# uricchio/2DSFS-scan

Measured on NVIDIA B200. Metric: SNPs/sec, 2D-SFS + T2D/T1D 20 kb window scan, higher is better.
Workload: dtype u32 popcount/histograms + f64 likelihoods

## Files before the change

2dsfs-scan_b200/csrc/tdsfs.cu:

```cuda
#include <algorithm>
#include <cmath>
#include <cstdarg>
#include <cstdio>
#include <cstdlib>
#include <cstring>
#include <string>
#include <vector>

#include <nvtx3/nvToolsExt.h>

#include "tdsfs_kernels.cuh"
#include "tdsfs_fused.cuh"

using namespace tdsfs;

#define TDSFS_VERSION 200

static thread_local std::string g_err;

struct NvtxRange {
  explicit NvtxRange(const char* name) { nvtxRangePushA(name); }
  ~NvtxRange() { nvtxRangePop(); }
};

// ... 70 lines not shown
  double* d_ws = nullptr;
  long long ws_cap = 0;
  long long fused_W = -1;
  int fused_snp = -1;
  bool ws_ready = false;
  bool last_fused = false;
  double* d_dxI = nullptr;
  int bg_mode = -1, NG = 0;
  long long gstride = 0;
  uint32_t* d_hist = nullptr;
  long long hist_words = 0;
  int32_t* d_bg_group = nullptr;
  int32_t* d_score_group = nullptr;
  bool per_chrom_scoring = false;
  double *d_lb2 = nullptr, *d_lb1a = nullptr, *d_lb1b = nullptr, *d_B = nullptr, *d_lnI = nullptr;
  unsigned long long* d_Bsum = nullptr;
  int table_groups = 0;
  bool float_bg = false, tables_ready = false, fin_timed = false;
  bool poisson_bg = false;
  double pq_n = 0, pq_sum = 0, pq_lnsum = 0;
  bool tables_from_exchange = false;
  unsigned int* d_gridbar = nullptr;
  unsigned long long* d_stamps = nullptr;
  bool want_tail_exchange = false;
  bool x_timed = false;
  int score_group_warps = 1;
  int* d_err = nullptr;
  int peer_rank = -1, peer_world = 0;
  uint32_t* peer_hist[PEER_MAX] = {};
  unsigned long long* peer_flags[PEER_MAX] = {};
  unsigned long long* d_peer_flags = nullptr;
  uint32_t* peer_exported_hist = nullptr;
  long long peer_words = 0;
  unsigned long long peer_epoch = 0;
  bool peer_ready = false;
  unsigned long long peer_pending = 0;
  long long ncand = 0, cand_cap = 0;
  std::vector<long long> cand_off_host;
  long long cand_W = -1;
  int cand_snp = -1;
  int groups_mode = -1, groups_chrom = -1;
  cudaStream_t plan_stream = nullptr;
  cudaEvent_t ev_fork = nullptr, ev_plan = nullptr, ev_plan0 = nullptr;
  long long plan_W = -1;
  int plan_snp = -1;
  bool planned_last = false;
// ... 78 lines not shown
  c->device = device;
  c->sm_count = prop.multiProcessorCount;
  CK(cudaStreamCreateWithFlags(&c->own_stream, cudaStreamNonBlocking));
  CK(cudaStreamCreateWithFlags(&c->copy_stream, cudaStreamNonBlocking));
  CK(cudaStreamCreateWithFlags(&c->plan_stream, cudaStreamNonBlocking));
  CK(cudaEventCreateWithFlags(&c->ev_fork, cudaEventDisableTiming));
  CK(cudaEventCreate(&c->ev_plan));
  CK(cudaEventCreate(&c->ev_plan0));
  c->stream = c->own_stream;
  for (int i = 0; i < NEV; ++i) CK(cudaEventCreate(&c->ev[i]));
  CKR(dev_alloc(&c->d_err, 1));
  CKR(dev_alloc(&c->d_nlarge, 1));
  CKR(dev_alloc(&c->d_lnI, LN_TABLE));
  CK(cudaMemsetAsync(c->d_err, 0, sizeof(int), c->stream));
  k_ln_int_table<<<(LN_TABLE + 255) / 256, 256, 0, c->stream>>>(c->d_lnI, LN_TABLE);
  c->launches++;
  CK(cudaGetLastError());
  CKR(dev_alloc(&c->d_gridbar, 2));
  CK(cudaMemsetAsync(c->d_gridbar, 0, 2 * sizeof(unsigned int), c->stream));
  if (getenv("TDSFS_TAIL_STAMPS")) {
    CKR(dev_alloc(&c->d_stamps, 8));
    CK(cudaMemsetAsync(c->d_stamps, 0, 8 * sizeof(unsigned long long), c->stream));
  }
  CKR(dev_alloc(&c->d_dxI, LN_TABLE));
  k_dx_table<<<(LN_TABLE + 255) / 256, 256, 0, c->stream>>>(c->d_dxI, LN_TABLE);
  c->launches++;
  CK(cudaGetLastError());
  CK(cudaStreamSynchronize(c->stream));
  *out = c;
  return 0;
}

static int pool_get(void** pool, size_t* cap, size_t bytes, void** out) {
  if (bytes > *cap) {
    if (*pool) cudaFree(*pool);
    *pool = nullptr;
    *cap = 0;
    CK(cudaMalloc(pool, std::max<size_t>(bytes, 256)));
    *cap = std::max<size_t>(bytes, 256);
  }
  *out = *pool;
  return 0;
}

static void drop_step_graph(tdsfs_ctx* c) {
  if (c->step_exec) cudaGraphExecDestroy(c->step_exec);
// ... 24 lines not shown
  if (!c) return;
  cudaSetDevice(c->device);
  cudaStreamSynchronize(c->stream);
  drop_step_graph(c);
  free_data(c);
  if (c->pool_G) cudaFree(c->pool_G);
  if (c->pool_cnt) cudaFree(c->pool_cnt);
  if (c->pool_pos) cudaFree(c->pool_pos);
  if (c->pool_flags) cudaFree(c->pool_flags);
  if (c->pool_off) cudaFree(c->pool_off);
  if (c->pool_tmp) cudaFree(c->pool_tmp);
  peer_unmap(c);
  dev_free(c->d_peer_flags);
  dev_free(c->d_work);
  if (c->d_rec) cudaFree(c->d_rec);
  dev_free(c->d_hist); dev_free(c->d_bg_group); dev_free(c->d_score_group);
  dev_free(c->d_lb2); dev_free(c->d_lb1a); dev_free(c->d_lb1b); dev_free(c->d_B); dev_free(c->d_Bsum); dev_free(c->d_lnI);
  dev_free(c->d_err); dev_free(c->d_cand_off); dev_free(c->d_wlo); dev_free(c->d_whi); dev_free(c->d_wchrom);
  dev_free(c->d_large); dev_free(c->d_wstart); dev_free(c->d_wend); dev_free(c->d_nlarge);
  dev_free(c->r_count); dev_free(c->r_n2); dev_free(c->r_n1a); dev_free(c->r_n1b); dev_free(c->r_T2); dev_free(c->r_T1a);
  dev_free(c->r_T1b); dev_free(c->r_flags); dev_free(c->d_scratch);
  for (int i = 0; i < NEV; ++i) if (c->ev[i]) cudaEventDestroy(c->ev[i]);
  dev_free(c->d_dxI); dev_free(c->d_ws); dev_free(c->d_gridbar); dev_free(c->d_stamps);
  cudaStreamDestroy(c->own_stream);
  cudaStreamDestroy(c->copy_stream);
  cudaStreamDestroy(c->plan_stream);
  cudaEventDestroy(c->ev_fork); cudaEventDestroy(c->ev_plan); cudaEventDestroy(c->ev_plan0);
  delete c;
}

extern "C" int tdsfs_set_stream(tdsfs_t* c, void* s) {
  if (!c) return fail(TDSFS_ERR_ARG, "ctx is NULL");
  c->stream = s ? (cudaStream_t)s : c->own_stream;
  drop_step_graph(c);
  return 0;
}

extern "C" int tdsfs_set_sync(tdsfs_t* c, int sync) {
  if (!c) return fail(TDSFS_ERR_ARG, "ctx is NULL");
  c->sync = sync != 0;
  return 0;
}

extern "C" int tdsfs_set_panel(tdsfs_t* c, int32_t n1, int32_t n2, int32_t fold) {
  if (!c) return fail(TDSFS_ERR_ARG, "ctx is NULL");
  if (n1 < 1 || n2 < 1 || n1 > 32767 || n2 > 32767) return fail(TDSFS_ERR_ARG, "panel sizes must be in [1, 32767] (got %d, %d)", n1, n2);
// ... 356 lines not shown
            dev_free(c->d_ws);
            CKR(dev_alloc(&c->d_ws, ncand * 4));
            c->ws_cap = ncand;
          }
          q.W = (uint32_t)c->plan_W;
          q.Wmagic = (uint32_t)std::min<unsigned long long>(0xFFFFFFFFull, (1ull << 32) / (unsigned long long)c->plan_W);
          q.cand_off = c->d_cand_off;
          q.ncand = ncand;
          q.ws = c->d_ws;
          q.dxI = c->d_dxI;
          q.lnI = c->d_lnI;
        } else {
          q.nw1 = q.nw2 = 0;
        }
        q.pos_tma = (((uintptr_t)c->dPos) & 15) == 0 && !getenv("TDSFS_NO_POS_TMA");
        q.snap_nearest = getenv("TDSFS_SNAP_BACK") ? 0 : 1;
        const int per_warp_fixed = q.tab_words * 4;
        while (depth > 1 && p.cwarps * (depth * (stage_stride + 8) + per_warp_fixed) + hist_words * 4 + 16 > smem_max) --depth;
        p.nstage = p.cwarps * depth;
        const int smem = p.nstage * stage_stride + p.cwarps * q.tab_words * 4 + ((p.nstage + 1) & ~1) * 8 + hist_words * 4;
        if (smem > smem_max) return fail(TDSFS_ERR_ARG, "count kernel geometry needs %d bytes of shared memory (warps %d, depth %d)", smem, p.cwarps, depth);
        const bool plain = !c->dFlags && c->nfix == 0 && p.bg_group == nullptr && p.bg_lo < 0 && c->fold && c->fmt.narrow &&
                           c->n1 >= 32 && c->n2 >= 32 && c->n1 <= 1023 && c->n2 <= 1023 && !getenv("TDSFS_NO_PLAIN");
        void (*kern)(FusedParams) = plain ? k1_fused<0, 0, true> : k1_fused<0, 0, false>;
        if (plain && c->W1 == 32 && c->W2 == 32) kern = k1_fused<32, 32, true>;
        else if (plain && c->W1 == 14 && c->W2 == 14) kern = k1_fused<14, 14, true>;
        CK(cudaFuncSetAttribute(kern, cudaFuncAttributeMaxDynamicSharedMemorySize, smem));
        const bool one_launch = c->chunks.size() == 1 && !c->chunks[0].ev && c->chunks[0].r1 > c->chunks[0].r0;
        const bool tail_x = c->want_tail_exchange && one_launch && mode != TDSFS_BG_NONE && NG == 1 && c->peer_ready &&
                            c->d_hist == c->peer_exported_hist && c->gstride == c->peer_words;
        const bool tail_fin = one_launch && mode != TDSFS_BG_NONE && !getenv("TDSFS_NO_TAIL") &&
                              (tail_x || (!c->want_tail_exchange && getenv("TDSFS_TAIL") != nullptr));
        if (tail_fin) {
          CKR(ensure_tables(c, NG));
          q.tail = tail_x ? 2 : 1;
          q.gridbar = c->d_gridbar;
          q.tail_timeout = PEER_TIMEOUT_CYCLES;
          q.stamps = c->d_stamps;
          FinParams& f = q.fin;
          f.hist = c->d_hist; f.gstride = c->gstride; f.NG = NG; f.bins2d = c->bins2d; f.R1 = c->R1; f.R2 = c->R2;
          f.n1 = c->n1; f.n2 = c->n2; f.lb2 = c->d_lb2; f.lb1a = c->d_lb1a; f.lb1b = c->d_lb1b; f.Bsum = c->d_Bsum; f.B = c->d_B;
          if (tail_x) {
            for (int r = 0; r < PEER_MAX; ++r) { q.peer.hist[r] = c->peer_hist[r]; q.peer.flags[r] = c->peer_flags[r]; }
            q.peer.rank = c->peer_rank; q.peer.world = c->peer_world; q.peer.words = c->peer_words; q.peer.err = c->d_err;
            q.peer.timeout_cycles = PEER_TIMEOUT_CYCLES;
            q.peer.ticket = reinterpret_cast<unsigned int*>(c->d_peer_flags + PEER_MAX);
            q.epoch_mem = c->d_peer_flags + PEER_MAX + 1;
            c->peer_epoch += 2;
          }
        }
        const long long tile_rows = (long long)p.tile_blocks * BLK;
        for (auto& ch : c->chunks) {
          if (ch.r1 <= ch.r0) continue;
          if (ch.ev) CK(cudaStreamWaitEvent(st, ch.ev, 0));
          p.r0 = ch.r0; p.r1 = ch.r1;
          const long long ntiles = (ch.r1 - ch.r0 + tile_rows - 1) / tile_rows;
          const int grid = (int)std::max<long long>(1, std::min<long long>((ntiles + p.cwarps - 1) / p.cwarps, (long long)c->sm_count));
          q.k = p;
          kern<<<grid, p.cwarps * 32, smem, st>>>(q);
          c->launches++;
        }
        if (fuse) {
          c->fused_W = c->plan_W;
          c->fused_snp = c->plan_snp;
          c->ws_ready = true;
        }
        if (tail_fin) {
          c->tables_ready = true;
          c->tables_from_exchange = true;
          c->fin_timed = false;
        }
      }
    }
  } else {
    p.r0 = 0; p.r1 = c->S;
    const long long ntiles = (c->S + K1C_THREADS - 1) / K1C_THREADS;
    if (ntiles > 0) {
      CK(cudaFuncSetAttribute(k1_counts, cudaFuncAttributeMaxDynamicSharedMemorySize, hist_bytes));
      const int grid = (int)std::min<long long>(ntiles, (long long)c->sm_count * 4);
      k1_counts<<<grid, K1C_THREADS, hist_bytes, st>>>(p);
      c->launches++;
    }
  }
// ... 730 lines not shown
    cudaEventElapsedTime(&c->ms[3], c->ev[EV_K2], c->ev[EV_K3S]);
    cudaEventElapsedTime(&c->ms[4], c->ev[EV_K3S], c->ev[EV_K3L]);
    cudaEventElapsedTime(&c->ms[6], c->ev[EV_SC0], c->ev[EV_K3L]);
    if (c->keys_ready) cudaEventElapsedTime(&c->ms[7], c->ev[EV_BG0], c->ev[EV_K3L]);
  }
  c->ms[5] = c->ms[0];
  if (c->x_timed) cudaEventElapsedTime(&c->ms[8], c->ev[EV_X0], c->ev[EV_X1]);
  cudaGetLastError();
  for (int i = 0; i < n && i < 10; ++i) ms[i] = c->ms[i];
  return 0;
}

extern "C" int64_t tdsfs_launch_count(tdsfs_t* c) { return c ? c->launches : 0; }

extern "C" int tdsfs_tail_stamps(tdsfs_t* c, uint64_t* out8) {
  if (!c || !out8) return fail(TDSFS_ERR_ARG, "ctx or out is NULL");
  if (!c->d_stamps) return fail(TDSFS_ERR_STATE, "tail stamps are off (create the handle with TDSFS_TAIL_STAMPS=1 set)");
  CK(cudaSetDevice(c->device));
  CK(cudaStreamSynchronize(c->stream));
  CK(cudaMemcpy(out8, c->d_stamps, 8 * sizeof(uint64_t), cudaMemcpyDeviceToHost));
  return 0;
}

extern "C" int tdsfs_scan_info(tdsfs_t* c, int32_t* fused, int32_t* record_bytes) {
  if (!c) return fail(TDSFS_ERR_ARG, "ctx is NULL");
  if (fused) *fused = c->last_fused ? 1 : 0;
  if (record_bytes) *record_bytes = c->fmt.narrow ? 4 : 8;
  return 0;
}
```

2dsfs-scan_b200/csrc/tdsfs_fused.cuh:

```cuda
#pragma once
#include <type_traits>

#include "tdsfs_kernels.cuh"

namespace tdsfs {

constexpr uint32_t WS_ONE_2D = 1u << 10, WS_ONE_1A = 1u << 11, WS_ONE_1B = 1u << 12, WS_NALL = 1u << 13;

struct FusedParams {
  KeyParams k;
  int wmode;
  uint32_t W, Wmagic;
  const long long* cand_off;
  long long ncand;
  double* ws;
  const double* dxI;
  const double* lnI;
  int pos_tma;
  int tab_words;
  int nw1, nw2;
  int snap_nearest;
  int tail;
  unsigned int* gridbar;
  long long tail_timeout;
  FinParams fin;
  PeerParams peer;
  unsigned long long* epoch_mem;
  unsigned long long* stamps;
};

__global__ void k_dx_table(double* t, int n) {
  int i = blockIdx.x * blockDim.x + threadIdx.x;
  if (i < n) t[i] = i ? log((double)i + 1.0) + (double)i * log1p(1.0 / (double)i) : 0.0;
}

__device__ __forceinline__ uint32_t udiv_magic(uint32_t x, uint32_t W, uint32_t M) {
  uint32_t qd = __umulhi(x, M);
  if (x - qd * W >= W) ++qd;
  return qd;
}

struct ChromWin {
  int c = -1, lo = 0, hi = -1;
  int cbase = 0;
  int nfull = 0;
};

__device__ __forceinline__ void chrom_win(const FusedParams& q, int s, ChromWin& cw) {
  if (s >= cw.lo && s < cw.hi) return;
  const KeyParams& p = q.k;
  int lo = 0, hi = p.C;
  while (hi - lo > 1) {
// ... 113 lines not shown
    hi[i] = blk[(2 * i + 1) * BLK];
    both[i] = lo[i] & hi[i];
  }
  const uint32_t c = popc_sum<P>(both);
  alt = popc_sum<P>(lo) + c;
  miss = popc_sum<P>(hi) - c;
}

__device__ __forceinline__ uint32_t fold_fast(int a, int n) {
  const uint32_t f = (uint32_t)min(a, 2 * n - a);
  return (f - 1u) < (uint32_t)(n - 1) ? f : 0u;
}

__device__ __forceinline__ void red_shared_inc_if(bool pr, const uint32_t* base, uint32_t idx) {
  asm volatile("{\n\t.reg .pred p;\n\tsetp.ne.u32 p, %0, 0;\n\t@p red.shared.add.u32 [%1], 1;\n\t}" ::"r"((uint32_t)pr), "r"(smem_u32(base) + idx * 4u) : "memory");
}
__device__ __forceinline__ void red_global_inc_if(bool pr, uint32_t* addr) {
  asm volatile("{\n\t.reg .pred p;\n\tsetp.ne.u32 p, %0, 0;\n\t@p red.global.add.u32 [%1], 1;\n\t}" ::"r"((uint32_t)pr), "l"(addr) : "memory");
}

template <int TW1, int TW2>
constexpr int k1f_max_warps() { return (TW1 + TW2) >= 48 ? 16 : K1_CWARPS; }

template <int TW1, int TW2, bool PLAIN>
__global__ void __launch_bounds__(k1f_max_warps<TW1, TW2>() * 32, 1) k1_fused(const __grid_constant__ FusedParams q) {
  const KeyParams& p = q.k;
  extern __shared__ __align__(128) uint8_t smem[];
  const int tid = threadIdx.x, lane = tid & 31;
  const int warp = __shfl_sync(0xffffffffu, tid >> 5, 0);
  const int W1 = TW1 > 0 ? TW1 : p.W1, W2 = TW2 > 0 ? TW2 : p.W2;
  const int RW = W1 + W2;
  const int tile_rows = p.tile_blocks * BLK;
  const int stage_stride = p.stage_bytes + tile_rows * 4;
  const int depth = p.nstage / p.cwarps;
  uint64_t* full = reinterpret_cast<uint64_t*>(smem + (size_t)p.nstage * stage_stride);
  SinkSmem sm;
  sm.corner = reinterpret_cast<uint32_t*>(full + ((p.nstage + 1) & ~1));
  sm.h1a = sm.corner + p.cr * p.cc;
  sm.h1b = sm.h1a + p.h1a;
  const int nhist = p.cr * p.cc + p.h1a + p.h1b;
  uint32_t* tab = sm.corner + ((nhist + 3) & ~3) + (size_t)warp * q.tab_words;
  uint32_t* w1a = tab + HASH_SLOTS;
  uint32_t* w1b = w1a + q.nw1;

  if (tid == 0) {
    for (int i = 0; i < p.nstage; ++i) mbar_init(full + i, 1);
    fence_barrier_init();
    if (q.stamps && blockIdx.x == 0) q.stamps[0] = (unsigned long long)clock64();
  }
  for (int i = tid; i < nhist; i += blockDim.x) sm.corner[i] = 0;
  if (q.wmode && warp < p.cwarps) {
    for (int i = lane; i < HASH_SLOTS; i += 32) tab[i] = EMPTY_KEY;
    for (int i = lane; i < q.nw1 + q.nw2; i += 32) w1a[i] = 0;
  }
  __syncthreads();

  const int r0 = (int)p.r0, r1 = (int)p.r1, S = (int)p.S;
  const int nparts = gridDim.x * p.cwarps;
  auto target = [&](int jj) -> int {
    if (jj <= 0) return r0;
    if (jj >= nparts) return r1;
    const long long t = r0 + (long long)(r1 - r0) * jj / nparts;
    return max(r0, (int)(t / tile_rows * tile_rows));
  };
  ChromCache cc;
  const int cta_group = PLAIN ? p.uniform_group : tile_group(p, target(blockIdx.x * p.cwarps), cc);

  if (warp < p.cwarps) {
    const int j = blockIdx.x * p.cwarps + warp;
    bool st0 = true, st1 = true, stl = true, sth = true;
    const int lo_clamp = r0 > 0 ? snap_row(q, r0, stl, lane, false) : 0;
    const int hi_clamp = r1 < S ? snap_row(q, r1, sth, lane, false) : S;
    int slo = lo_clamp, shi = hi_clamp;
    if (j > 0) {
      slo = snap_row(q, target(j), st0, lane, q.snap_nearest != 0);
      if (slo <= lo_clamp) { slo = lo_clamp; st0 = stl; }
      if (slo >= hi_clamp) { slo = hi_clamp; st0 = sth; }
    } else {
      st0 = stl;
    }
    if (j + 1 < nparts) {
      shi = snap_row(q, target(j + 1), st1, lane, q.snap_nearest != 0);
      if (shi <= lo_clamp) shi = lo_clamp;
      if (shi >= hi_clamp) shi = hi_clamp;
    }
    slo = __shfl_sync(0xffffffffu, slo, 0);
    shi = __shfl_sync(0xffffffffu, shi, 0);
    st0 = __shfl_sync(0xffffffffu, (int)st0, 0) != 0;
    if (slo < shi) {
      uint8_t* stages = smem + (size_t)warp * depth * stage_stride;
      uint64_t* bars = full + warp * depth;
      const long long block_words = (long long)RW * BLK;
      const int b_end = (r1 + BLK - 1) / BLK;
      const int S4 = S & ~3;
      const int t_begin = slo / tile_rows, t_end = (shi - 1) / tile_rows + 1;
      const int t_whole = min(b_end, S4 / BLK) / p.tile_blocks;
      const uint32_t gbytes_whole = (uint32_t)(p.tile_blocks * block_words * 4);
      const uint32_t pbytes_whole = q.pos_tma ? (uint32_t)tile_rows * 4u : 0u;
      auto issue = [&](int t, int slot) {
        const int blk0 = t * p.tile_blocks;
        uint32_t gbytes = gbytes_whole, pbytes = pbytes_whole;
        if (t >= t_whole) {
          const int nb = min(p.tile_blocks, b_end - blk0);
          gbytes = (uint32_t)(nb * block_words * 4);
          pbytes = q.pos_tma ? (uint32_t)max(0, min(nb * BLK, S4 - blk0 * BLK)) * 4u : 0u;
        }
        uint8_t* stage = stages + (size_t)slot * stage_stride;
        mbar_arrive_expect_tx(bars + slot, gbytes + pbytes);
        bulk_g2s_stream(stage, p.G + (long long)blk0 * block_words, gbytes, bars + slot);
        if (pbytes) bulk_g2s(stage + p.stage_bytes, p.pos + (long long)blk0 * BLK, pbytes, bars + slot);
      };
      if (lane == 0)
        for (int d = 0; d < depth; ++d)
          if (t_begin + d < t_end) issue(t_begin + d, d);
      int slot = 0;
      uint32_t ph = 0;

      int cur_id = -2;
      bool overflow = false;
      bool pending_skip = !st0;
      int wcount = 0;
      int win_end_pos = 0, win_end_row = 0;
      double w2 = 0.0;
      uint32_t nn = 0;
      uint32_t aux = 0;
      ChromWin cw;
      const uint32_t last = (uint32_t)p.bins2d - 1;
      constexpr uint32_t F10 = (1u << KEY_SHIFT) - 1;

      auto close_window = [&]() {
        __syncwarp();
        if (cur_id >= 0) {
          if (!overflow) {
            double a1 = 0.0, b1 = 0.0;
            uint32_t dd = 0;
            for (int i = lane; i < q.nw1; i += 32) {
              const uint32_t v = w1a[i];
// ... 76 lines not shown
          int pv = 0;
          if (live) {
            const uint32_t* rowp = tile + (size_t)b * block_words + lane;
            if constexpr (TW1 > 0 && TW2 > 0) {
              count_pop_planes<TW1>(rowp, T1, M1);
              count_pop_planes<TW2>(rowp + TW1 * BLK, T2, M2);
              T1 += M1;
              T2 += M2;
            } else {
              count_block_b32<TW1>(rowp, W1, T1, M1);
              count_block_b32<TW2>(rowp + W1 * BLK, W2, T2, M2);
            }
            if (q.wmode == 1 && q.pos_tma) {
              if (INTERIOR || s < S4) pv = spos[b * BLK + lane];
              else if (s < S) pv = __ldg(p.pos + s);
            }
          }
          if (q.wmode == 1 && !q.pos_tma) {
            pv = pv_next;
            pv_next = s + BLK < S ? __ldg(p.pos + s + BLK) : 0;
          }
          if (b == nb - 1) {
            __syncwarp();
            if (lane == 0 && t + depth < t_end) {
              fence_proxy_async();
              issue(t + depth, slot);
            }
          }
          if (!live) return;
          const bool whole = INTERIOR || (sb >= slo && sb + BLK <= shi);
          const bool act = whole || (s >= slo && s < shi);
          uint32_t key = 0, fa = 0, fb = 0, cf = 1;
          if (act) {
            const int alt1 = (int)(T1 - M1), alt2 = (int)(T2 - M2);
            const int ref1 = 2 * (p.ns1 - (int)M1) - alt1, ref2 = 2 * (p.ns2 - (int)M2) - alt2;
            if (PLAIN) {
              const bool swapped = alt1 + alt2 > p.n1 + p.n2;
              const int k1 = swapped ? ref1 : alt1, k2 = swapped ? ref2 : alt2;
              int d1 = swapped ? (p.n1 - p.ns1) + (int)M1 : 0, d2 = swapped ? (p.n2 - p.ns2) + (int)M2 : 0;
              if ((d1 | d2) >> p.fmt.md) {
                atomicOr(p.err, 8);
                d1 = d2 = 0;
              }
              key = (uint32_t)(k1 * p.C2 + k2);
              __stcs(reinterpret_cast<uint32_t*>(p.rec) + s,
                     (uint32_t)k1 | ((uint32_t)k2 << p.fmt.b1) | ((uint32_t)d1 << (p.fmt.b1 + p.fmt.b2)) |
                         ((uint32_t)d2 << (p.fmt.b1 + p.fmt.b2 + p.fmt.md)));
              fa = fold_fast(alt1, p.n1);
              fb = fold_fast(alt2, p.n2);
// ... 41 lines not shown
              if (wcount > WCAP) overflow = true;
              else if (mine) insert(key, fa, fb, cf);
            }
          }
          {
            const uint32_t am = __ballot_sync(0xffffffffu, act);
            const int src = 31 - __clz((int)am);
            const int c_lo = __shfl_sync(0xffffffffu, cw.lo, src), c_hi = __shfl_sync(0xffffffffu, cw.hi, src);
            const int c_base = __shfl_sync(0xffffffffu, cw.cbase, src);
            if (cur_id < 0) {
              win_end_pos = 0;
              win_end_row = 0;
            } else if (q.wmode == 1) {
              const long long e = 1 + (long long)(cur_id - c_base + 1) * (long long)q.W;
              win_end_pos = e > 0x7FFFFFFFLL ? 0x7FFFFFFF : (int)e;
              win_end_row = c_hi;
            } else {
              win_end_pos = 0x7FFFFFFF;
              win_end_row = c_lo + (cur_id - c_base + 1) * (int)q.W;
            }
          }
      };

      for (int t = t_begin; t < t_end; ++t) {
        const int blk0 = t * p.tile_blocks;
        const int nb = min(p.tile_blocks, b_end - blk0);
        mbar_wait(bars + slot, ph);
        const uint8_t* stage = stages + (size_t)slot * stage_stride;
        const uint32_t* tile = reinterpret_cast<const uint32_t*>(stage);
        const int* spos = reinterpret_cast<const int*>(stage + p.stage_bytes);
        if (blk0 * BLK >= slo && (blk0 + nb) * BLK <= shi) {
          for (int b = 0; b < nb; ++b) do_block(std::true_type{}, t, blk0, nb, b, tile, spos);
        } else {
          for (int b = 0; b < nb; ++b) do_block(std::false_type{}, t, blk0, nb, b, tile, spos);
        }
        if (++slot == depth) { slot = 0; ph ^= 1; }
      }
      if (q.wmode) close_window();
    }
  }
  __syncthreads();
  sink_flush(p, sm, cta_group, tid, blockDim.x);
  if (q.tail) {
    auto stamp = [&](int i) { if (q.stamps && blockIdx.x == 0 && tid == 0) q.stamps[i] = (unsigned long long)clock64(); };
    stamp(1);
    grid_barrier(q.gridbar, p.err, q.tail_timeout);
    stamp(2);
    if (q.tail == 2) peer_exchange(q.peer, q.epoch_mem, q.stamps);
    for (int g = 0; g < q.fin.NG; ++g) finalize_tables(q.fin, g, blockIdx.x, gridDim.x);
    stamp(6);
    finalize_totals(q.fin, gridDim.x);
    stamp(7);
  }
}

struct FinishParams {
  ScoreParams s;
  const double* ws;
  int use_smem;
  int large_ctas;
};

__device__ __forceinline__ uint32_t bin_of(const uint2 r, int which, uint32_t last) {
  if (which == 0) return (r.x != 0 && r.x != last) ? r.x : 0u;
// ... 89 lines not shown
    auto lookup1 = [&](uint32_t rr, double& la, double& lb) {
      const uint32_t k1 = rr & m1, k2 = (rr >> sh2) & m2;
      la = s_a[k1 + 2u * ((rr >> shd1) & md)];
      lb = s_b[k2 + 2u * (rr >> shd2)];
    };
    {
      constexpr int Q = 8;
      auto bounds = [&](long long w, int& lo, int& cnt) {
        lo = 0; cnt = 0;
        if (w < p.ncand) {
          lo = __ldg(p.wlo + w);
          const int c = __ldg(p.whi + w) - lo;
          cnt = c <= WCAP ? c : 0;
        }
      };
      auto load_batch = [&](uint32_t (&r)[Q], int lo, int cnt, int base) {
#pragma unroll
        for (int j = 0; j < Q; ++j) {
          const int i = base + j * 32 + lane;
          r[j] = i < cnt ? __ldcs(rec + lo + i) : 0u;
        }
      };
      double g2 = 0.0, g1a = 0.0, g1b = 0.0;
      auto consume = [&](const uint32_t (&r)[Q]) {
#pragma unroll
        for (int h4 = 0; h4 < Q; h4 += 4) {
          double l2[4], la[4], lb[4];
#pragma unroll
          for (int j = 0; j < 4; ++j) {
            l2[j] = lookup2(r[h4 + j]);
            lookup1(r[h4 + j], la[j], lb[j]);
          }
#pragma unroll
          for (int j = 0; j < 4; ++j) { g2 += l2[j]; g1a += la[j]; g1b += lb[j]; }
        }
      };
      long long id = wid, nid = wid + nwarp;
      int lo, cnt, nlo, ncnt;
      bounds(id, lo, cnt);
      bounds(nid, nlo, ncnt);
      uint32_t rn[Q];
      load_batch(rn, lo, cnt, 0);
      while (id < p.ncand) {
        uint32_t r[Q], r2[Q];
#pragma unroll
        for (int j = 0; j < Q; ++j) r[j] = rn[j];
        if (cnt > Q * 32) load_batch(r2, lo, cnt, Q * 32);
        const long long nnid = nid + nwarp;
        int nnlo, nncnt;
        bounds(nnid, nnlo, nncnt);
        load_batch(rn, nlo, ncnt, 0);
        if (cnt > 0) {
          const double wsv = __ldg(q.ws + id * 4 + (lane & 3));
          g2 = g1a = g1b = 0.0;
          consume(r);
          if (cnt > Q * 32) consume(r2);
          if (cnt > 2 * Q * 32) {
            load_batch(r2, lo, cnt, 2 * Q * 32);
            consume(r2);
          }
          g2 = warp_sum(g2); g1a = warp_sum(g1a); g1b = warp_sum(g1b);
          finish_window(p, id, lo, cnt, g2, g1a, g1b, wsv, p.lb2, p.lb1a, p.lb1b, p.B, lane);
        }
        id = nid; lo = nlo; cnt = ncnt;
        nid = nnid; nlo = nnlo; ncnt = nncnt;
      }
    }
  } else {
    for (long long id = wid; id < p.ncand; id += nwarp) {
      const int lo = __ldg(p.wlo + id), hi = __ldg(p.whi + id);
      const int cnt = hi - lo;
      if (cnt == 0 || cnt > WCAP) continue;
      const int g = p.score_group ? __ldg(p.score_group + __ldg(p.wchrom + id)) : 0;
      const double* lb2 = p.lb2 + (long long)g * p.bins2d;
      const double* lb1a = p.lb1a + (long long)g * (p.n1 + 1);
      const double* lb1b = p.lb1b + (long long)g * (p.n2 + 1);
      double g2 = 0.0, g1a = 0.0, g1b = 0.0;
      constexpr int Q = 4;
      for (int base = 0; base < cnt; base += Q * 32) {
        uint2 r[Q];
        double l2[Q], la[Q], lb[Q];
#pragma unroll
// ... 24 lines not shown
```

2dsfs-scan_b200/tdsfs_capi.py:

```python
from __future__ import annotations

import ctypes as C
import os

import numpy as np

HERE = os.path.dirname(os.path.abspath(__file__))
LIB_PATH = os.path.join(HERE, "lib", "libtdsfs.so")

BG_NONE, BG_PER_CHROM, BG_GENOME, BG_CHROM = 0, 1, 2, 3
F_T2D_NONE, F_T1D_P1_NONE, F_T1D_P2_NONE, F_EMPTY, F_SKIPPED = 1, 2, 4, 8, 16
ERR_ARG, ERR_CUDA, ERR_STATE, ERR_RANGE, ERR_RETRY = 1, 2, 3, 4, 5

EXPORTS = [
    "tdsfs_create", "tdsfs_destroy", "tdsfs_last_error", "tdsfs_set_stream", "tdsfs_set_sync", "tdsfs_set_panel",
    "tdsfs_load_counts", "tdsfs_load_genotypes", "tdsfs_background", "tdsfs_background_device", "tdsfs_get_background",
    "tdsfs_set_background", "tdsfs_finalize_background", "tdsfs_plan_bp", "tdsfs_plan_snp", "tdsfs_candidates_bp", "tdsfs_candidates_snp", "tdsfs_scan_bp",
    "tdsfs_scan_snp", "tdsfs_set_poisson_background", "tdsfs_scan_poisson_bp", "tdsfs_fetch_results", "tdsfs_check", "tdsfs_run_bp", "tdsfs_step_bp", "tdsfs_window_spectra", "tdsfs_likelihood",
    "tdsfs_poisson_score", "tdsfs_peer_export", "tdsfs_peer_import", "tdsfs_peer_allreduce_background", "tdsfs_peer_reduce_finalize", "tdsfs_peer_close",
    "tdsfs_synth_genotypes", "tdsfs_timings", "tdsfs_launch_count", "tdsfs_scan_info", "tdsfs_tail_stamps", "tdsfs_version",
]


PEER_BLOB_BYTES = 192


class TdsfsError(RuntimeError):
    def __init__(self, code, msg):
        super().__init__(f"libtdsfs error {code}: {msg}")
        self.code = code


class Fixup(C.Structure):
    _fields_ = [("snp", C.c_int64), ("pop", C.c_int32), ("dref", C.c_int32), ("dalt", C.c_int32)]


FIXUP_DTYPE = np.dtype([("snp", "<i8"), ("pop", "<i4"), ("dref", "<i4"), ("dalt", "<i4")], align=True)


class Result(C.Structure):
    _fields_ = [("chrom", C.c_void_p), ("start", C.c_void_p), ("end", C.c_void_p), ("snp_count", C.c_void_p),
                ("n2d", C.c_void_p), ("n1d_p1", C.c_void_p), ("n1d_p2", C.c_void_p), ("T2D", C.c_void_p),
                ("T1D_p1", C.c_void_p), ("T1D_p2", C.c_void_p), ("flags", C.c_void_p)]
# ... 228 lines not shown
        self._check(self._L.tdsfs_synth_genotypes(self._h, C.c_void_p(G_dev_ptr), C.c_int64(S), C.c_int64(snp0), C.c_int32(words1),
                                                  C.c_int32(words2), C.c_int32(ns1), C.c_int32(ns2), C.c_uint64(seed),
                                                  C.c_double(missing_rate), C.c_double(fst)))

    def timings(self):
        ms = (C.c_float * 10)()
        self._check(self._L.tdsfs_timings(self._h, ms, C.c_int32(10)))
        names = ["k1_count", "finalize", "k2_bounds", "k3_small", "k3_large", "background_call", "scan_call", "pass_total", "exchange"]
        return dict(zip(names, list(ms)))

    def launch_count(self):
        return int(self._L.tdsfs_launch_count(self._h))

    def scan_info(self):
        f, b = C.c_int32(), C.c_int32()
        self._check(self._L.tdsfs_scan_info(self._h, C.byref(f), C.byref(b)))
        return bool(f.value), int(b.value)

    def tail_stamps(self):
        out = (C.c_uint64 * 8)()
        self._check(self._L.tdsfs_tail_stamps(self._h, out))
        return [int(x) for x in out]

    def check(self):
        self._check(self._L.tdsfs_check(self._h))
```

include/tdsfs.h:

```cpp
#ifndef TDSFS_H
#define TDSFS_H

#include <stdint.h>

#ifdef __cplusplus
extern "C" {
#endif

typedef struct tdsfs_ctx tdsfs_t;

enum {
  TDSFS_OK = 0,
  TDSFS_ERR_ARG = 1,
  TDSFS_ERR_CUDA = 2,
  TDSFS_ERR_STATE = 3,
  TDSFS_ERR_RANGE = 4,
  TDSFS_ERR_RETRY = 5
};

enum {
  TDSFS_F_T2D_NONE = 1,
  TDSFS_F_T1D_P1_NONE = 2,
  TDSFS_F_T1D_P2_NONE = 4,
  TDSFS_F_EMPTY = 8,
// ... 71 lines not shown
int tdsfs_fetch_results(tdsfs_t* ctx, tdsfs_result_t* out, int64_t cap, int64_t* n_windows);

int tdsfs_check(tdsfs_t* ctx);

int tdsfs_run_bp(tdsfs_t* ctx, int32_t bg_mode, int64_t W, tdsfs_result_t* out, int64_t cap, int64_t* n_windows);

int tdsfs_set_poisson_background(tdsfs_t* ctx, const double* q2d);
int tdsfs_scan_poisson_bp(tdsfs_t* ctx, int64_t W, tdsfs_result_t* out, int64_t cap, int64_t* n_windows);

int tdsfs_step_bp(tdsfs_t* ctx, int32_t bg_mode, int64_t W);

int tdsfs_window_spectra(tdsfs_t* ctx, int64_t window, uint64_t* sfs2d, uint64_t* sfs1d_p1, uint64_t* sfs1d_p2);

int tdsfs_likelihood(tdsfs_t* ctx, const int64_t* x, const double* b, int64_t n, double B, double* T, int32_t* flag);

int tdsfs_poisson_score(tdsfs_t* ctx, const int64_t* x, const double* mu, int64_t n, double* score);

int tdsfs_synth_genotypes(tdsfs_t* ctx, void* G_dev, int64_t S, int64_t snp0, int32_t words1, int32_t words2,
                          int32_t ns1, int32_t ns2, uint64_t seed, double missing_rate, double fst);
int tdsfs_timings(tdsfs_t* ctx, float* ms, int32_t n);
int64_t tdsfs_launch_count(tdsfs_t* ctx);
int tdsfs_scan_info(tdsfs_t* ctx, int32_t* fused, int32_t* record_bytes);
int tdsfs_tail_stamps(tdsfs_t* ctx, uint64_t* out8);
int tdsfs_version(void);

#ifdef __cplusplus
}
#endif
#endif
```

Baseline: 22.42 billion.

## Add dynamic tail work-stealing to fused count kernel via atomic chunk pool

The fused count kernel now splits its row range into a static part (about 85% by default) that is divided evenly across warps, plus a pool of shrinking chunks that warps claim through a global atomic counter once their static range is done. Chunk bounds are snapped to window boundaries and cached in a tagged global array, and the next chunk's first tile is prefetched at the end of the current one. A per-launch epoch counter resets the pool. The aim is to cut load imbalance at the tail of the scan, at the cost of extra atomics, window-state resets and a second kernel instantiation. The likelihood consume loop also skips unused batch groups, and optional per-CTA timing stamps are added for profiling.

```diff
diff --git a/2dsfs-scan_b200/csrc/tdsfs.cu b/2dsfs-scan_b200/csrc/tdsfs.cu
--- a/2dsfs-scan_b200/csrc/tdsfs.cu
+++ b/2dsfs-scan_b200/csrc/tdsfs.cu
@@ -116,6 +116,11 @@
   bool tables_from_exchange = false;
   unsigned int* d_gridbar = nullptr;
   unsigned long long* d_stamps = nullptr;
+  unsigned int* d_k1dyn = nullptr;
+  unsigned long long* d_k1bnd = nullptr;
+  long long k1bnd_cap = 0;
+  unsigned long long* d_cta_stamps = nullptr;
+  int cta_stamps_n = 0;
   bool want_tail_exchange = false;
   bool x_timed = false;
   int score_group_warps = 1;
@@ -240,6 +245,12 @@
     CKR(dev_alloc(&c->d_stamps, 8));
     CK(cudaMemsetAsync(c->d_stamps, 0, 8 * sizeof(unsigned long long), c->stream));
   }
+  CKR(dev_alloc(&c->d_k1dyn, 4));
+  CK(cudaMemsetAsync(c->d_k1dyn, 0, 4 * sizeof(unsigned int), c->stream));
+  if (getenv("TDSFS_K1_STAMPS")) {
+    CKR(dev_alloc(&c->d_cta_stamps, 2 * (long long)c->sm_count));
+    CK(cudaMemsetAsync(c->d_cta_stamps, 0, 2 * (size_t)c->sm_count * sizeof(unsigned long long), c->stream));
+  }
   CKR(dev_alloc(&c->d_dxI, LN_TABLE));
   k_dx_table<<<(LN_TABLE + 255) / 256, 256, 0, c->stream>>>(c->d_dxI, LN_TABLE);
   c->launches++;
@@ -310,6 +321,7 @@
   dev_free(c->r_T1b); dev_free(c->r_flags); dev_free(c->d_scratch);
   for (int i = 0; i < NEV; ++i) if (c->ev[i]) cudaEventDestroy(c->ev[i]);
   dev_free(c->d_dxI); dev_free(c->d_ws); dev_free(c->d_gridbar); dev_free(c->d_stamps);
+  dev_free(c->d_k1dyn); dev_free(c->d_k1bnd); dev_free(c->d_cta_stamps);
   cudaStreamDestroy(c->own_stream);
   cudaStreamDestroy(c->copy_stream);
   cudaStreamDestroy(c->plan_stream);
@@ -712,10 +724,16 @@
         if (smem > smem_max) return fail(TDSFS_ERR_ARG, "count kernel geometry needs %d bytes of shared memory (warps %d, depth %d)", smem, p.cwarps, depth);
         const bool plain = !c->dFlags && c->nfix == 0 && p.bg_group == nullptr && p.bg_lo < 0 && c->fold && c->fmt.narrow &&
                            c->n1 >= 32 && c->n2 >= 32 && c->n1 <= 1023 && c->n2 <= 1023 && !getenv("TDSFS_NO_PLAIN");
-        void (*kern)(FusedParams) = plain ? k1_fused<0, 0, true> : k1_fused<0, 0, false>;
-        if (plain && c->W1 == 32 && c->W2 == 32) kern = k1_fused<32, 32, true>;
-        else if (plain && c->W1 == 14 && c->W2 == 14) kern = k1_fused<14, 14, true>;
-        CK(cudaFuncSetAttribute(kern, cudaFuncAttributeMaxDynamicSharedMemorySize, smem));
+        void (*kerns[2])(FusedParams) = {plain ? k1_fused<0, 0, true, false> : k1_fused<0, 0, false, false>,
+                                         plain ? k1_fused<0, 0, true, true> : k1_fused<0, 0, false, true>};
+        if (plain && c->W1 == 32 && c->W2 == 32) {
+          kerns[0] = k1_fused<32, 32, true, false>;
+          kerns[1] = k1_fused<32, 32, true, true>;
+        } else if (plain && c->W1 == 14 && c->W2 == 14) {
+          kerns[0] = k1_fused<14, 14, true, false>;
+          kerns[1] = k1_fused<14, 14, true, true>;
+        }
+        for (auto kn : kerns) CK(cudaFuncSetAttribute(kn, cudaFuncAttributeMaxDynamicSharedMemorySize, smem));
         const bool one_launch = c->chunks.size() == 1 && !c->chunks[0].ev && c->chunks[0].r1 > c->chunks[0].r0;
         const bool tail_x = c->want_tail_exchange && one_launch && mode != TDSFS_BG_NONE && NG == 1 && c->peer_ready &&
                             c->d_hist == c->peer_exported_hist && c->gstride == c->peer_words;
@@ -740,15 +758,50 @@
           }
         }
         const long long tile_rows = (long long)p.tile_blocks * BLK;
+        constexpr double K1_DYN_MIN_WINDOWS = 16.0;
+        const char* e_static = getenv("TDSFS_K1_STATIC");
+        const int k1_mode = depth != 1 ? 1 : (e_static ? (atoi(e_static) != 0 ? 1 : 0) : -1);
+        const long long ncand_all = q.wmode ? c->cand_off_host[c->C] : 0;
+        double static_frac = 0.85;
+        if (const char* e = getenv("TDSFS_K1_STATIC_FRAC")) static_frac = std::max(0.0, std::min(1.0, atof(e)));
+        int chunk_tiles = 0;
+        if (const char* e = getenv("TDSFS_K1_CHUNK")) chunk_tiles = std::max(0, atoi(e));
+        q.cta_stamps = c->d_cta_stamps;
         for (auto& ch : c->chunks) {
           if (ch.r1 <= ch.r0) continue;
           if (ch.ev) CK(cudaStreamWaitEvent(st, ch.ev, 0));
           p.r0 = ch.r0; p.r1 = ch.r1;
           const long long ntiles = (ch.r1 - ch.r0 + tile_rows - 1) / tile_rows;
           const int grid = (int)std::max<long long>(1, std::min<long long>((ntiles + p.cwarps - 1) / p.cwarps, (long long)c->sm_count));
+          q.pool_lo = (int)ch.r1;
+          q.nchunk = 0;
+          q.chunk_tiles = chunk_tiles;
+          const double rows_per_win = ncand_all > 0 ? (double)c->S / (double)ncand_all : 0.0;
+          const double win_per_warp = rows_per_win > 0.0 ? (double)(ch.r1 - ch.r0) / rows_per_win / ((double)grid * p.cwarps) : 0.0;
+          if (k1_mode == 0 || (k1_mode < 0 && win_per_warp >= K1_DYN_MIN_WINDOWS)) {
+            const long long pool_lo = std::max<long long>(ch.r0, (ch.r0 + (long long)(static_frac * (double)(ch.r1 - ch.r0))) / tile_rows * tile_rows);
+            const long long pool_tiles = (ch.r1 - pool_lo + tile_rows - 1) / tile_rows;
+            long long m = std::min<long long>(pool_tiles, 2LL * grid * p.cwarps);
+            if (rows_per_win > 0.0) m = std::min<long long>(m, std::max<long long>(1, (long long)((double)(ch.r1 - pool_lo) / (4.0 * rows_per_win))));
+            if (chunk_tiles > 0) m = (pool_tiles + chunk_tiles - 1) / chunk_tiles;
+            if (m > 0 && pool_lo < ch.r1) {
+              if (m + 1 > c->k1bnd_cap) {
+                CK(cudaStreamSynchronize(st));
+                dev_free(c->d_k1bnd);
+                CKR(dev_alloc(&c->d_k1bnd, m + 1));
+                CK(cudaMemsetAsync(c->d_k1bnd, 0, (size_t)(m + 1) * sizeof(unsigned long long), st));
+                c->k1bnd_cap = m + 1;
+              }
+              q.pool_lo = (int)pool_lo;
+              q.nchunk = (int)m;
+            }
+          }
+          q.dyn = c->d_k1dyn;
+          q.bnd = c->d_k1bnd;
           q.k = p;
-          kern<<<grid, p.cwarps * 32, smem, st>>>(q);
+          kerns[q.nchunk > 0 ? 1 : 0]<<<grid, p.cwarps * 32, smem, st>>>(q);
           c->launches++;
+          c->cta_stamps_n = grid;
         }
         if (fuse) {
           c->fused_W = c->plan_W;
@@ -1525,6 +1578,16 @@
   return 0;
 }
 
+extern "C" int tdsfs_k1_stamps(tdsfs_t* c, uint64_t* out, int n) {
+  if (!c || !out) return fail(TDSFS_ERR_ARG, "ctx or out is NULL");
+  if (!c->d_cta_stamps) return fail(TDSFS_ERR_STATE, "count-kernel stamps are off (create the handle with TDSFS_K1_STAMPS=1 set)");
+  CK(cudaSetDevice(c->device));
+  CK(cudaStreamSynchronize(c->stream));
+  const int k = std::min(n, c->cta_stamps_n);
+  if (k > 0) CK(cudaMemcpy(out, c->d_cta_stamps, 2 * (size_t)k * sizeof(uint64_t), cudaMemcpyDeviceToHost));
+  return k;
+}
+
 extern "C" int tdsfs_scan_info(tdsfs_t* c, int32_t* fused, int32_t* record_bytes) {
   if (!c) return fail(TDSFS_ERR_ARG, "ctx is NULL");
   if (fused) *fused = c->last_fused ? 1 : 0;
diff --git a/2dsfs-scan_b200/csrc/tdsfs_fused.cuh b/2dsfs-scan_b200/csrc/tdsfs_fused.cuh
--- a/2dsfs-scan_b200/csrc/tdsfs_fused.cuh
+++ b/2dsfs-scan_b200/csrc/tdsfs_fused.cuh
@@ -27,7 +27,19 @@
   PeerParams peer;
   unsigned long long* epoch_mem;
   unsigned long long* stamps;
+  int pool_lo;
+  int nchunk;
+  int chunk_tiles;
+  unsigned int* dyn;
+  unsigned long long* bnd;
+  unsigned long long* cta_stamps;
 };
+
+__device__ __forceinline__ unsigned long long global_timer() {
+  unsigned long long t;
+  asm volatile("mov.u64 %0, %%globaltimer;" : "=l"(t));
+  return t;
+}
 
 __global__ void k_dx_table(double* t, int n) {
   int i = blockIdx.x * blockDim.x + threadIdx.x;
@@ -187,7 +199,7 @@
 template <int TW1, int TW2>
 constexpr int k1f_max_warps() { return (TW1 + TW2) >= 48 ? 16 : K1_CWARPS; }
 
-template <int TW1, int TW2, bool PLAIN>
+template <int TW1, int TW2, bool PLAIN, bool DYN>
 __global__ void __launch_bounds__(k1f_max_warps<TW1, TW2>() * 32, 1) k1_fused(const __grid_constant__ FusedParams q) {
   const KeyParams& p = q.k;
   extern __shared__ __align__(128) uint8_t smem[];
@@ -212,6 +224,7 @@
     for (int i = 0; i < p.nstage; ++i) mbar_init(full + i, 1);
     fence_barrier_init();
     if (q.stamps && blockIdx.x == 0) q.stamps[0] = (unsigned long long)clock64();
+    if (q.cta_stamps) q.cta_stamps[2 * blockIdx.x] = global_timer();
   }
   for (int i = tid; i < nhist; i += blockDim.x) sm.corner[i] = 0;
   if (q.wmode && warp < p.cwarps) {
@@ -221,12 +234,21 @@
   __syncthreads();
 
   const int r0 = (int)p.r0, r1 = (int)p.r1, S = (int)p.S;
+  const int pool_lo = DYN ? q.pool_lo : r1;
   const int nparts = gridDim.x * p.cwarps;
   auto target = [&](int jj) -> int {
     if (jj <= 0) return r0;
-    if (jj >= nparts) return r1;
-    const long long t = r0 + (long long)(r1 - r0) * jj / nparts;
+    if (jj >= nparts) return pool_lo;
+    const long long t = r0 + (long long)(pool_lo - r0) * jj / nparts;
     return max(r0, (int)(t / tile_rows * tile_rows));
+  };
+  auto chunk_row = [&](int k) -> int {
+    const int m = q.nchunk;
+    if (k >= m) return r1;
+    long long t;
+    if (q.chunk_tiles > 0) t = pool_lo + (long long)k * q.chunk_tiles * tile_rows;
+    else t = pool_lo + (long long)(r1 - pool_lo) * ((long long)k * (7LL * m - 3LL * k)) / (4LL * m * m);
+    return min(r1, max(pool_lo, (int)(t / tile_rows * tile_rows)));
   };
   ChromCache cc;
   const int cta_group = PLAIN ? p.uniform_group : tile_group(p, target(blockIdx.x * p.cwarps), cc);
@@ -236,29 +258,58 @@
     bool st0 = true, st1 = true, stl = true, sth = true;
     const int lo_clamp = r0 > 0 ? snap_row(q, r0, stl, lane, false) : 0;
     const int hi_clamp = r1 < S ? snap_row(q, r1, sth, lane, false) : S;
-    int slo = lo_clamp, shi = hi_clamp;
-    if (j > 0) {
-      slo = snap_row(q, target(j), st0, lane, q.snap_nearest != 0);
-      if (slo <= lo_clamp) { slo = lo_clamp; st0 = stl; }
-      if (slo >= hi_clamp) { slo = hi_clamp; st0 = sth; }
-    } else {
-      st0 = stl;
-    }
-    if (j + 1 < nparts) {
-      shi = snap_row(q, target(j + 1), st1, lane, q.snap_nearest != 0);
-      if (shi <= lo_clamp) shi = lo_clamp;
-      if (shi >= hi_clamp) shi = hi_clamp;
-    }
+    auto bound = [&](int nominal, bool& st) -> int {
+      if (nominal <= r0) { st = stl; return lo_clamp; }
+      if (nominal >= r1) { st = sth; return hi_clamp; }
+      int v = snap_row(q, nominal, st, lane, q.snap_nearest != 0);
+      if (v <= lo_clamp) { v = lo_clamp; st = stl; }
+      if (v >= hi_clamp) { v = hi_clamp; st = sth; }
+      return v;
+    };
+    int slo = bound(target(j), st0), shi = bound(target(j + 1), st1);
     slo = __shfl_sync(0xffffffffu, slo, 0);
     shi = __shfl_sync(0xffffffffu, shi, 0);
     st0 = __shfl_sync(0xffffffffu, (int)st0, 0) != 0;
+
+    constexpr bool dyn = DYN;
+    const uint32_t tag = dyn ? __ldcg(q.dyn + 2) + 1u : 0u;
+    auto chunk_bound = [&](int k, bool& st) -> int {
+      unsigned long long e = lane == 0 ? __ldcg(q.bnd + k) : 0ull;
+      e = __shfl_sync(0xffffffffu, e, 0);
+      if ((uint32_t)(e >> 32) == tag) {
+        st = (e & 1ull) != 0;
+        return (int)((uint32_t)e >> 1);
+      }
+      const int v = bound(chunk_row(k), st);
+      if (lane == 0) __stcg(q.bnd + k, (unsigned long long)tag << 32 | (unsigned long long)((uint32_t)v << 1 | (st ? 1u : 0u)));
+      return v;
+    };
+    int nlo = 0, nhi = 0;
+    bool nst = true;
+    auto claim = [&]() {
+      nlo = nhi = 0;
+      if (!dyn) return;
+      while (true) {
+        int k = lane == 0 ? (int)atomicAdd(q.dyn, 1u) : 0;
+        k = __shfl_sync(0xffffffffu, k, 0);
+        if (k >= q.nchunk) return;
+        bool st_hi;
+        const int lo = chunk_bound(k, nst), hi = chunk_bound(k + 1, st_hi);
+        if (lo < hi) { nlo = lo; nhi = hi; return; }
+      }
+    };
+    if (slo >= shi) {
+      claim();
+      slo = nlo; shi = nhi; st0 = nst;
+      nlo = nhi = 0;
+    }
     if (slo < shi) {
       uint8_t* stages = smem + (size_t)warp * depth * stage_stride;
       uint64_t* bars = full + warp * depth;
       const long long block_words = (long long)RW * BLK;
       const int b_end = (r1 + BLK - 1) / BLK;
       const int S4 = S & ~3;
-      const int t_begin = slo / tile_rows, t_end = (shi - 1) / tile_rows + 1;
+      int t_begin = slo / tile_rows, t_end = (shi - 1) / tile_rows + 1;
       const int t_whole = min(b_end, S4 / BLK) / p.tile_blocks;
       const uint32_t gbytes_whole = (uint32_t)(p.tile_blocks * block_words * 4);
       const uint32_t pbytes_whole = q.pos_tma ? (uint32_t)tile_rows * 4u : 0u;
@@ -278,6 +329,11 @@
       if (lane == 0)
         for (int d = 0; d < depth; ++d)
           if (t_begin + d < t_end) issue(t_begin + d, d);
+      if (dyn)
+        for (int k = j; k <= q.nchunk; k += nparts) {
+          bool st;
+          chunk_bound(k, st);
+        }
       int slot = 0;
       uint32_t ph = 0;
 
@@ -400,9 +456,17 @@
           }
           if (b == nb - 1) {
             __syncwarp();
-            if (lane == 0 && t + depth < t_end) {
-              fence_proxy_async();
-              issue(t + depth, slot);
+            if (t + depth < t_end) {
+              if (lane == 0) {
+                fence_proxy_async();
+                issue(t + depth, slot);
+              }
+            } else if (dyn) {
+              claim();
+              if (lane == 0 && nlo < nhi) {
+                fence_proxy_async();
+                issue(nlo / tile_rows, slot);
+              }
             }
           }
           if (!live) return;
@@ -490,24 +554,50 @@
           }
       };
 
-      for (int t = t_begin; t < t_end; ++t) {
-        const int blk0 = t * p.tile_blocks;
-        const int nb = min(p.tile_blocks, b_end - blk0);
-        mbar_wait(bars + slot, ph);
-        const uint8_t* stage = stages + (size_t)slot * stage_stride;
-        const uint32_t* tile = reinterpret_cast<const uint32_t*>(stage);
-        const int* spos = reinterpret_cast<const int*>(stage + p.stage_bytes);
-        if (blk0 * BLK >= slo && (blk0 + nb) * BLK <= shi) {
-          for (int b = 0; b < nb; ++b) do_block(std::true_type{}, t, blk0, nb, b, tile, spos);
-        } else {
-          for (int b = 0; b < nb; ++b) do_block(std::false_type{}, t, blk0, nb, b, tile, spos);
-        }
-        if (++slot == depth) { slot = 0; ph ^= 1; }
+      while (true) {
+        for (int t = t_begin; t < t_end; ++t) {
+          const int blk0 = t * p.tile_blocks;
+          const int nb = min(p.tile_blocks, b_end - blk0);
+          mbar_wait(bars + slot, ph);
+          const uint8_t* stage = stages + (size_t)slot * stage_stride;
+          const uint32_t* tile = reinterpret_cast<const uint32_t*>(stage);
+          const int* spos = reinterpret_cast<const int*>(stage + p.stage_bytes);
+          if (blk0 * BLK >= slo && (blk0 + nb) * BLK <= shi) {
+            for (int b = 0; b < nb; ++b) do_block(std::true_type{}, t, blk0, nb, b, tile, spos);
+          } else {
+            for (int b = 0; b < nb; ++b) do_block(std::false_type{}, t, blk0, nb, b, tile, spos);
+          }
+          if (++slot == depth) { slot = 0; ph ^= 1; }
+        }
+        if (q.wmode) close_window();
+        if (nlo >= nhi) break;
+        slo = __shfl_sync(0xffffffffu, nlo, 0);
+        shi = __shfl_sync(0xffffffffu, nhi, 0);
+        pending_skip = !nst;
+        nlo = nhi = 0;
+        cur_id = -2;
+        overflow = false;
+        win_end_pos = win_end_row = 0;
+        t_begin = slo / tile_rows;
+        t_end = (shi - 1) / tile_rows + 1;
+        if (q.wmode == 1 && !q.pos_tma) {
+          const int s_first = t_begin * tile_rows + lane;
+          pv_next = s_first < S ? __ldg(p.pos + s_first) : 0;
+        }
       }
-      if (q.wmode) close_window();
     }
   }
   __syncthreads();
+  if (DYN && tid == 0) {
+    __threadfence();
+    if (atomicAdd(q.dyn + 1, 1u) == gridDim.x - 1) {
+      atomicExch(q.dyn, 0u);
+      atomicExch(q.dyn + 1, 0u);
+      atomicAdd(q.dyn + 2, 1u);
+      __threadfence();
+    }
+  }
+  if (q.cta_stamps && tid == 0) q.cta_stamps[2 * blockIdx.x + 1] = global_timer();
   sink_flush(p, sm, cta_group, tid, blockDim.x);
   if (q.tail) {
     auto stamp = [&](int i) { if (q.stamps && blockIdx.x == 0 && tid == 0) q.stamps[i] = (unsigned long long)clock64(); };
@@ -643,14 +733,20 @@
         }
       };
       double g2 = 0.0, g1a = 0.0, g1b = 0.0;
-      auto consume = [&](const uint32_t (&r)[Q]) {
+      auto consume = [&](const uint32_t (&r)[Q], int left) {
+        const int ng = min(Q, (left + 31) >> 5);
 #pragma unroll
         for (int h4 = 0; h4 < Q; h4 += 4) {
+          if (h4 >= ng) break;
           double l2[4], la[4], lb[4];
 #pragma unroll
           for (int j = 0; j < 4; ++j) {
-            l2[j] = lookup2(r[h4 + j]);
-            lookup1(r[h4 + j], la[j], lb[j]);
+            if (h4 + j < ng) {
+              l2[j] = lookup2(r[h4 + j]);
+              lookup1(r[h4 + j], la[j], lb[j]);
+            } else {
+              l2[j] = la[j] = lb[j] = 0.0;
+            }
           }
 #pragma unroll
           for (int j = 0; j < 4; ++j) { g2 += l2[j]; g1a += la[j]; g1b += lb[j]; }
@@ -674,11 +770,11 @@
         if (cnt > 0) {
           const double wsv = __ldg(q.ws + id * 4 + (lane & 3));
           g2 = g1a = g1b = 0.0;
-          consume(r);
-          if (cnt > Q * 32) consume(r2);
+          consume(r, cnt);
+          if (cnt > Q * 32) consume(r2, cnt - Q * 32);
           if (cnt > 2 * Q * 32) {
             load_batch(r2, lo, cnt, 2 * Q * 32);
-            consume(r2);
+            consume(r2, cnt - 2 * Q * 32);
           }
           g2 = warp_sum(g2); g1a = warp_sum(g1a); g1b = warp_sum(g1b);
           finish_window(p, id, lo, cnt, g2, g1a, g1b, wsv, p.lb2, p.lb1a, p.lb1b, p.B, lane);
diff --git a/2dsfs-scan_b200/tdsfs_capi.py b/2dsfs-scan_b200/tdsfs_capi.py
--- a/2dsfs-scan_b200/tdsfs_capi.py
+++ b/2dsfs-scan_b200/tdsfs_capi.py
@@ -18,7 +18,7 @@
     "tdsfs_set_background", "tdsfs_finalize_background", "tdsfs_plan_bp", "tdsfs_plan_snp", "tdsfs_candidates_bp", "tdsfs_candidates_snp", "tdsfs_scan_bp",
     "tdsfs_scan_snp", "tdsfs_set_poisson_background", "tdsfs_scan_poisson_bp", "tdsfs_fetch_results", "tdsfs_check", "tdsfs_run_bp", "tdsfs_step_bp", "tdsfs_window_spectra", "tdsfs_likelihood",
     "tdsfs_poisson_score", "tdsfs_peer_export", "tdsfs_peer_import", "tdsfs_peer_allreduce_background", "tdsfs_peer_reduce_finalize", "tdsfs_peer_close",
-    "tdsfs_synth_genotypes", "tdsfs_timings", "tdsfs_launch_count", "tdsfs_scan_info", "tdsfs_tail_stamps", "tdsfs_version",
+    "tdsfs_synth_genotypes", "tdsfs_timings", "tdsfs_launch_count", "tdsfs_scan_info", "tdsfs_tail_stamps", "tdsfs_k1_stamps", "tdsfs_version",
 ]
 
 
@@ -293,5 +293,12 @@
         self._check(self._L.tdsfs_tail_stamps(self._h, out))
         return [int(x) for x in out]
 
+    def k1_stamps(self, n=1024):
+        out = (C.c_uint64 * (2 * n))()
+        k = self._L.tdsfs_k1_stamps(self._h, out, n)
+        if k < 0:
+            self._check(k)
+        return [(int(out[2 * i]), int(out[2 * i + 1])) for i in range(k)]
+
     def check(self):
         self._check(self._L.tdsfs_check(self._h))
diff --git a/include/tdsfs.h b/include/tdsfs.h
--- a/include/tdsfs.h
+++ b/include/tdsfs.h
@@ -117,6 +117,7 @@
 int64_t tdsfs_launch_count(tdsfs_t* ctx);
 int tdsfs_scan_info(tdsfs_t* ctx, int32_t* fused, int32_t* record_bytes);
 int tdsfs_tail_stamps(tdsfs_t* ctx, uint64_t* out8);
+int tdsfs_k1_stamps(tdsfs_t* ctx, uint64_t* out, int n);
 int tdsfs_version(void);
 
 #ifdef __cplusplus
```

Result: faster. 22.75 billion (median of 6 runs) (+1.5%).
